# bioinfomaticsCSU/deepsignal

Hardware: AMD Instinct MI355X
Metric: CpG sites/sec (batch=512, k=17, sig=360) (higher is better)
Workload: dtype f32; 1 GPU; configs[1]: 1xMI355X, batch=512, random-init CpG model weights, synthetic (17,360) features, fp32; batch=512, kmer_len=17, signal_len=360

## Files before the change

deepsignal_amd/csrc/ds_engine.cpp:

```cpp
#include "../../include/deepsignal_hip.h"
#include "ds_internal.h"
#include "ds_extract.h"
#include "ds_tsv_device.h"
#include "ds_freq.h"
#include "ds_combine.h"
#include "ds_eval.h"
#include "ds_train.h"
#include "ds_train_signal.h"

#include <algorithm>
#include <cmath>
#include <cstdio>
#include <cstdlib>
#include <cstring>
#include <functional>
#include <map>
#include <string>
#include <vector>

using namespace ds;

namespace {

constexpr int VOCAB = 1024, EMB = 128, HID = 256, NLAYER = 3, NMOD = 11, INC_OUT = 240;
// ... 3 lines not shown

void same_pad(int in, int k, int s, int* out, int* pl)
{
    int o = (in + s - 1) / s;
    int tot = std::max((o - 1) * s + k - in, 0);
    *out = o;
    *pl = tot / 2;
}

struct HostTensor {
    std::vector<int64_t> shape;
    std::vector<float> data;
};

struct PackedGemm {
    float* Bp = nullptr;
    float* bias = nullptr;
    int K = 0, N = 0;
    float* Bps = nullptr;
    float* Bp16 = nullptr;
};

enum OpKind { OP_GEMM, OP_STEM1, OP_MAXPOOL, OP_AVGPOOL, OP_HEAD, OP_FUSED, OP_PACKEV, OP_LSTM, OP_STEM23, OP_HEADF, OP_DENSES, OP_XPROJ };
enum Operands { OPS_FP32, OPS_BF16, OPS_SPLIT };
constexpr KernelClass kFusedKernels[3][3] = {{K_FUSED1, K_FUSED2, K_FUSED3}, {K_FUSEDB1, K_FUSEDB2, K_FUSEDB3}, {K_FUSEDS1, K_FUSEDS2, K_FUSEDS3}};
constexpr KernelClass kStem23Kernels[3] = {K_STEM23, K_STEM23B, K_STEM23S};

struct GemmOp { GemmCfg cfg; int launch_index, total_tiles; };
struct Stem1Op { const float* signals; float* out; };
struct PoolOp { const float* in; float* out; int win, wout, pad, ch; };
struct LstmDiagOp { int launch_index; LstmTile tile; };

struct Op {
    OpKind kind;
    KernelClass kernel;
    Operands operands = OPS_FP32;
    int stream;
    int stage;
    bool after_join = false;
    GemmOp gemm{};
    Stem1Op stem1{};
    PoolOp pool{};
    LstmDiagOp lstm{};
    FusedChain fc{};
    int tm = 0;
    Stem23Args sa{};
    HeadFoldedArgs ha{};
    SplitDense sd{};
    LstmXproj xp{};
    double flops = 0;
    hipEvent_t ev0 = nullptr, ev1 = nullptr;
    bool pending = false;
    int run_launches = 0;
    double run_flops = 0;
};

#define DS_KERNEL_NAME(id, name) name,
const char* const kKernelNames[K_COUNT] = {DS_KERNEL_TABLE(DS_KERNEL_NAME)};
#undef DS_KERNEL_NAME
struct KernelStat {
    int64_t launches = 0;
    double total_ms = 0;
    double flops = 0;
};

struct Stage {
    std::string name;
    int stream = 0;
    int launches = 0;
    double flops_per_site = 0;
    double total_ms = 0;
    int64_t calls = 0;
};

#define DS_SPLIT_DENSE_PARTS 4

struct Plan {
    int n = 0;
    std::vector<GemmLaunch> launches;
    GemmLaunch* d_launches = nullptr;
    std::vector<LstmLaunch> lstm_launches;
    std::vector<Op> ops;
    int fc1_parts = 1;
    hipGraphExec_t graph = nullptr;
    int64_t uses = 0, last_use = 0;
};

enum class Ticket { Idle, Forward, Text, Rows };
using dss::Times;

template <class R>
struct TableRuns {
    R* open = nullptr;
    typename R::Tally ended;
    void close()
    {
        if (!open) return;
        ended.add(open->t);
        delete open;
        open = nullptr;
    }
};
struct Block { char* p = nullptr; size_t cap = 0; };

}

struct Slot {
    hipStream_t s0 = nullptr, s1 = nullptr;
    bool owns_s1 = true;
    hipEvent_t ev_fork = nullptr, ev_join = nullptr;
    float* d_in = nullptr;
    int* d_kmer = nullptr;
    float *d_means = nullptr, *d_stds = nullptr, *d_sanums = nullptr, *d_signals = nullptr;
    float *stem_pool = nullptr, *conv2o = nullptr, *conv3o = nullptr;
    float* modout[NMOD] = {nullptr};
    float *pool2 = nullptr, *pool3 = nullptr;
    float *tmpA = nullptr, *tmpS = nullptr, *tmpB = nullptr;
    float* sigfeat = nullptr;
    float* H[2][NLAYER] = {{nullptr}};
    float* Cst[2][NLAYER] = {{nullptr}};
    float* xproj[2] = {nullptr, nullptr};
    float* hlast[2] = {nullptr, nullptr};
    float *fc1o = nullptr, *logits = nullptr, *act = nullptr;
    int* pred = nullptr;
    float* joint = nullptr;
    char* jsplit = nullptr;

    Ticket ticket = Ticket::Idle;
    int submitted_n = 0;
    char* pin_in = nullptr;
    float* pin_act = nullptr;
    int* pin_pred = nullptr;
    Block pin_reads, d_reads;
    Block d_rows, pin_rows;
    int64_t* pin_rowoff = nullptr;
    char* d_rc = nullptr;
    int* pin_rc = nullptr;
    hipEvent_t rc_ev[2] = {nullptr, nullptr};
    bool rc_selected = false;
    bool rc_timed = false;
    char *pin_text = nullptr, *d_text = nullptr;
    int32_t *d_tres = nullptr, *pin_tres = nullptr;
    hipEvent_t tx_ev[5] = {nullptr, nullptr, nullptr, nullptr, nullptr};
    std::vector<std::pair<const char*, const char*>> text_rows;

    std::map<int, Plan> plans;
    int last_n = 0;
    int last_fc1_parts = 1;
};

#ifndef DS_SPLIT_DENSE_MIN_N
#define DS_SPLIT_DENSE_MIN_N 1
#endif
struct ds_handle {
    ds_config cfg{};
    std::string err;
    int T = 17, S = 360, C = 2;
    int w1 = 0, wa = 0, wb = 0, wc = 0, J = 0, SF = 0;
    int pl_conv1 = 0, pl_pool1 = 0, pl_pool2 = 0, pl_pool3 = 0;
    int B = 512;
    bool is_cnn = true, is_rnn = true, is_base = true;
    bool bf16 = false;
    bool split_dense_narrow = false;
    bool lstm_xproj = false;
    bool lstm_xproj_all = false;
    int split_dense_min_n = DS_SPLIT_DENSE_MIN_N;
    bool split = false;
// ... 942 lines not shown
            if (h->is_rnn) {
                add_seg(G, h->cur->hlast[0], HID, 0, HID);
                add_seg(G, h->cur->hlast[1], HID, 0, HID);
            }
            if (h->is_cnn) add_seg(G, h->cur->sigfeat, h->SF, 0, h->SF);
        }
        add_out(G, h->cur->fc1o, h->J, 0, h->J, 0);
        add_tiles(L, G, fc_cfg);
        P.add_gemm_op(P.tail, st, fc_cfg, L, bf ? (double)h->J / h->JP : 1.0);
    }
    Op op = make_op(OP_HEAD, K_HEAD, 0, stage_id(h, "head", 0));
    op.flops = 2.0 * h->J * h->C * n;
    P.add_op(P.tail, op);
}

int build_plan(ds_handle* h, int n, Plan* plan)
{
    plan->n = n;
    Planner P{h, plan, n, !h->stages_done, h->bf16};
    if (h->is_cnn) plan_signal_model(P);
    plan_event_model(P);
    plan_joint_model(P);

    size_t i = 0, j = 0;
    while (i < P.cnn.size() || j < P.rnn.size()) {
        if (i < P.cnn.size()) plan->ops.push_back(P.cnn[i++]);
        if (j < P.rnn.size()) plan->ops.push_back(P.rnn[j++]);
    }
    for (Op& op : P.tail) { op.after_join = true; plan->ops.push_back(op); }

    void* p = nullptr;
    const auto& LS = plan->launches;
    HIPCHK(h, hipMalloc(&p, LS.size() * sizeof(GemmLaunch)));
    h->allocs.push_back(p);
    plan->d_launches = static_cast<GemmLaunch*>(p);
    HIPCHK(h, hipMemcpy(p, LS.data(), LS.size() * sizeof(GemmLaunch), hipMemcpyHostToDevice));
    return DS_OK;
}

int issue_op(ds_handle* h, Plan& plan, const Op& op, hipStream_t s)
{
    const int n = plan.n;
    const bool bf_rows = op.operands == OPS_BF16;
    switch (op.kind) {
    case OP_GEMM: HIPCHK(h, launch_gemm(op.gemm.cfg, plan.d_launches + op.gemm.launch_index, op.gemm.total_tiles, s)); break;
    case OP_STEM1: HIPCHK(h, launch_stem1(op.stem1.signals, h->stem1_w, h->stem1_b, op.stem1.out, n, h->S, h->w1, h->pl_conv1, h->wa, h->pl_pool1, bf_rows, s)); break;
    case OP_MAXPOOL:
        if (bf_rows) HIPCHK(h, launch_maxpool_s2_bf16(op.pool.in, op.pool.out, n, op.pool.win, op.pool.wout, op.pool.pad, op.pool.ch, s));
        else HIPCHK(h, launch_maxpool_s2(op.pool.in, op.pool.out, n, op.pool.win, op.pool.wout, op.pool.pad, op.pool.ch, s));
        break;
    case OP_AVGPOOL:
        if (bf_rows) HIPCHK(h, launch_avgpool7_bf16(op.pool.in, op.pool.out, n, op.pool.win, op.pool.ch, 256, h->JP, h->is_rnn ? 2 * HID : 0, s));
        else HIPCHK(h, launch_avgpool7(op.pool.in, op.pool.out, n, op.pool.win, op.pool.ch, s));
        break;
    case OP_PACKEV: HIPCHK(h, launch_pack_event_feat_bf16(h->cur->hlast[0], h->cur->hlast[1], h->cur->joint, n, h->JP, 0, s)); break;
    case OP_LSTM:
        if (lstm_tile_is_split(op.lstm.tile)) HIPCHK(h, launch_lstm_cells_split(op.lstm.tile, h->terms, plan.lstm_launches[op.lstm.launch_index], s));
        else HIPCHK(h, launch_lstm_cells(op.lstm.tile, plan.lstm_launches[op.lstm.launch_index], s));
        break;
    case OP_DENSES: HIPCHK(h, launch_dense_split(h->terms, op.sd, s)); break;
    case OP_XPROJ: HIPCHK(h, launch_lstm_xproj(h->terms, op.xp, s)); break;
    case OP_STEM23:
        switch (op.operands) {
        case OPS_FP32: HIPCHK(h, launch_stem23(op.sa, s)); break;
        case OPS_BF16: HIPCHK(h, launch_stem23_bf16(op.sa, s)); break;
        case OPS_SPLIT: HIPCHK(h, launch_stem23_split(h->terms, op.sa, s)); break;
        }
        break;
    case OP_HEADF: HIPCHK(h, launch_head_folded(op.ha, s)); break;
    case OP_FUSED:
        switch (op.operands) {
        case OPS_FP32: HIPCHK(h, launch_inception_fused(op.tm, op.fc, s)); break;
        case OPS_BF16: HIPCHK(h, launch_inception_fused_bf16(op.tm, op.fc, s)); break;
        case OPS_SPLIT: HIPCHK(h, launch_inception_fused_split(h->terms, op.tm, op.fc, s)); break;
        }
        break;
    case OP_HEAD:
        HIPCHK(h, launch_head(h->cur->fc1o, h->fc2, h->cur->logits, h->cur->act, h->cur->pred, n, h->J, h->C, s, plan.fc1_parts, (size_t)h->B * h->J));
        break;
    }
    return DS_OK;
}

int enqueue_forward(ds_handle* h, Plan& plan, int timed)
{
    HIPCHK(h, hipEventRecord(h->cur->ev_fork, h->cur->s0));
    HIPCHK(h, hipStreamWaitEvent(h->cur->s1, h->cur->ev_fork, 0));
    bool joined = false;
    const bool serial = h->serial || timed == 3;
    if (timed == 3) timed = 1;
    Op* head[2] = {nullptr, nullptr};
    auto close_run = [&](int si) -> int {
        if (head[si]) {
            HIPCHK(h, hipEventRecord(head[si]->ev1, si == 0 ? h->cur->s0 : h->cur->s1));
            head[si]->pending = true;
            head[si] = nullptr;
        }
        return DS_OK;
    };
    for (Op& op : plan.ops) {
        const int si = (op.stream == 0 || serial) ? 0 : 1;
        hipStream_t s = si == 0 ? h->cur->s0 : h->cur->s1;
        if (op.after_join && !joined) {
            int rc = close_run(0); if (rc) return rc;
            rc = close_run(1); if (rc) return rc;
            HIPCHK(h, hipEventRecord(h->cur->ev_join, h->cur->s1));
            HIPCHK(h, hipStreamWaitEvent(h->cur->s0, h->cur->ev_join, 0));
            joined = true;
        }
        if (timed && !op.ev0) {
            HIPCHK(h, hipEventCreate(&op.ev0));
            HIPCHK(h, hipEventCreate(&op.ev1));
        }
        if (timed == 2) {
            HIPCHK(h, hipEventRecord(op.ev0, s));
            op.run_launches = 1; op.run_flops = op.flops;
        } else if (timed == 1) {
            if (head[si] && head[si]->kernel != op.kernel) { int rc = close_run(si); if (rc) return rc; }
            if (!head[si]) {
                head[si] = &op;
                op.run_launches = 0; op.run_flops = 0;
                HIPCHK(h, hipEventRecord(op.ev0, s));
            }
            head[si]->run_launches += 1;
            head[si]->run_flops += op.flops;
        }
        int rc = issue_op(h, plan, op, s);
        if (rc) return rc;
        if (timed == 2) {
            HIPCHK(h, hipEventRecord(op.ev1, s));
            op.pending = true;
        }
    }
    { int rc = close_run(0); if (rc) return rc; rc = close_run(1); if (rc) return rc; }
    if (!joined) {
        HIPCHK(h, hipEventRecord(h->cur->ev_join, h->cur->s1));
        HIPCHK(h, hipStreamWaitEvent(h->cur->s0, h->cur->ev_join, 0));
    }
    return DS_OK;
}

int collect_stage_times(ds_handle* h)
{
    for (Slot& sl : h->slots)
      for (auto& kv : sl.plans)
        for (Op& op : kv.second.ops) {
            if (!op.pending) continue;
            HIPCHK(h, hipEventSynchronize(op.ev1));
            float ms = 0;
            HIPCHK(h, hipEventElapsedTime(&ms, op.ev0, op.ev1));
            h->stages[op.stage].total_ms += ms;
            KernelStat& K = h->kstat[op.kernel];
            K.launches += op.run_launches; K.total_ms += ms; K.flops += op.run_flops;
            op.pending = false;
        }
    return DS_OK;
}

void destroy_plan(ds_handle* h, Plan& p)
{
    if (p.graph) hipGraphExecDestroy(p.graph);
    for (Op& op : p.ops) { if (op.ev0) hipEventDestroy(op.ev0); if (op.ev1) hipEventDestroy(op.ev1); }
    if (p.d_launches) {
        hipFree(p.d_launches);
        auto it = std::find(h->allocs.begin(), h->allocs.end(), (void*)p.d_launches);
        if (it != h->allocs.end()) h->allocs.erase(it);
    }
    p.graph = nullptr; p.d_launches = nullptr; p.ops.clear();
}

constexpr size_t MAX_PLANS_PER_SLOT = 24;

int get_plan(ds_handle* h, int n, Plan** out)
{
    auto& plans = h->cur->plans;
    auto it = plans.find(n);
    if (it == plans.end()) {
        if (plans.size() >= MAX_PLANS_PER_SLOT && !h->profiling) {
            auto victim = plans.end();
            for (auto jt = plans.begin(); jt != plans.end(); ++jt)
                if (jt->first != h->B && (victim == plans.end() || jt->second.last_use < victim->second.last_use)) victim = jt;
            if (victim != plans.end()) {
                HIPCHK(h, hipStreamSynchronize(h->cur->s0));
                HIPCHK(h, hipStreamSynchronize(h->cur->s1));
                destroy_plan(h, victim->second);
                plans.erase(victim);
            }
        }
        Plan p;
        int rc = build_plan(h, n, &p);
        if (rc) return rc;
        it = plans.emplace(n, std::move(p)).first;
        h->stages_done = true;
    }
    it->second.uses += 1;
    it->second.last_use = ++h->plan_tick;
    *out = &it->second;
    return DS_OK;
}

int ensure_graph(ds_handle* h, Plan& plan)
{
    if (plan.graph) return DS_OK;
    hipGraph_t g = nullptr;
    HIPCHK(h, hipStreamBeginCapture(h->cur->s0, hipStreamCaptureModeThreadLocal));
    int rc = enqueue_forward(h, plan, 0);
    hipError_t e = hipStreamEndCapture(h->cur->s0, &g);
    if (rc) { if (g) hipGraphDestroy(g); return rc; }
    if (e != hipSuccess) return fail(h, DS_ERR_HIP, std::string("hipStreamEndCapture: ") + hipGetErrorString(e));
    e = hipGraphInstantiate(&plan.graph, g, nullptr, nullptr, 0);
    hipGraphDestroy(g);
    if (e != hipSuccess) return fail(h, DS_ERR_HIP, std::string("hipGraphInstantiate: ") + hipGetErrorString(e));
    return DS_OK;
}

int run_resident(ds_handle* h, int n)
{
    Plan* plan = nullptr;
    int rc = get_plan(h, n, &plan);
    if (rc) return rc;
    h->cur->last_n = n;
    h->cur->last_fc1_parts = plan->fc1_parts;
    if (h->profiling) {
        rc = collect_stage_times(h);
        if (rc) return rc;
        rc = enqueue_forward(h, *plan, h->profiling);
        if (rc) return rc;
        for (Stage& S : h->stages) S.calls += 1;
        return DS_OK;
    }
    if (h->use_graph && (plan->graph || n == h->B || plan->uses >= 2)) {
        rc = ensure_graph(h, *plan);
        if (rc) return rc;
        HIPCHK(h, hipGraphLaunch(plan->graph, h->cur->s0));
        return DS_OK;
    }
    return enqueue_forward(h, *plan, 0);
}

void prepare_slots(ds_handle* h)
{
    if (!h->use_graph || h->debug || h->serial) return;
    Slot* keep = h->cur;
    const std::string err_before = h->err;
    for (Slot& sl : h->slots) {
        h->cur = &sl;
        Plan* plan = nullptr;
        int rc = get_plan(h, h->B, &plan);
        if (!rc) { plan->uses = 0; rc = ensure_graph(h, *plan); }
        if (rc) {
            fprintf(stderr, "deepsignal_amd: preparing a slot's full-batch plan failed (%s); plans will be built at the first forward\n",
                    h->err.c_str());
            h->err = err_before;
            break;
        }
    }
    h->cur = keep;
}

}

namespace {
template <class F>
auto guarded(ds_handle* h, F&& body) -> decltype(body())
{
    try {
        return body();
    } catch (const std::bad_alloc&) {
        return fail(h, DS_ERR_NOMEM, "out of host memory");
    } catch (const std::exception& e) {
        return fail(h, DS_ERR_INVALID, std::string("internal error: ") + e.what());
    } catch (...) {
        return fail(h, DS_ERR_INVALID, "internal error");
    }
}

template <class R, class Begin>
int open_run(ds_handle* h, TableRuns<R> ds_handle::*runs, const char* call, Begin begin)
{
    if (!h) return DS_ERR_INVALID;
    TableRuns<R>& r = h->*runs;
    if (r.open) return fail(h, DS_ERR_INVALID, std::string(R::ROUTE) + "_" + call + ": a run is open on this handle (" + R::ROUTE + "_end first)");
    r.open = new R();
    std::string err;
    const int rc = begin(*r.open, &err);
    if (rc == DS_OK) return DS_OK;
    delete r.open;
    r.open = nullptr;
    return fail(h, rc, err);
}

template <class R, class Call>
auto in_run(ds_handle* h, TableRuns<R> ds_handle::*runs, const char* call, Call body, const char* opener = "begin")
    -> decltype(body(std::declval<R&>(), (std::string*)nullptr))
{
    if (!h) return DS_ERR_INVALID;
    R* r = (h->*runs).open;
    if (!r) return fail(h, DS_ERR_INVALID, std::string(R::ROUTE) + "_" + call + ": no run is open (" + R::ROUTE + "_" + opener + " first)");
    std::string err;
    const auto rc = body(*r, &err);
    return rc < 0 ? fail(h, (int)rc, err) : rc;
}

template <class R>
int end_run(ds_handle* h, TableRuns<R> ds_handle::*runs)
{
    if (!h) return DS_ERR_INVALID;
    (h->*runs).close();
    return DS_OK;
}
}

extern "C" {

const char* ds_version(void)
{
    return "deepsignal_amd 0.5 (gfx950; fp32 MFMA, bf16 conv + FC and bf16_all operand modes; bf16x3 = fp32 operands as three bf16 "
           "terms, six products per MAC, in: conv_layer2 / 3, the eleven inception modules, the BiLSTM cells' recurrent and lower-layer products, dense(J, J) of the three-step "
           "joint model; fp16x2 = the same scope on two fp16 terms, three products per MAC, operands within +-65504)";
}

const char* ds_last_error(const ds_handle* h) { return h ? h->err.c_str() : g_create_error.c_str(); }

static int ds_create_impl(const ds_config* cfg, ds_handle** out)
{
    if (!cfg || !out) return fail(nullptr, DS_ERR_INVALID, "ds_create: null argument");
    *out = nullptr;
    if (!(cfg->is_cnn || cfg->is_rnn))
        return fail(nullptr, DS_ERR_INVALID, "at least one of is_cnn/is_rnn should be True");
    if (cfg->precision != DS_PRECISION_FP32 && cfg->precision != DS_PRECISION_BF16 && cfg->precision != DS_PRECISION_BF16_ALL &&
        cfg->precision != DS_PRECISION_BF16X3 && cfg->precision != DS_PRECISION_FP16X2)
        return fail(nullptr, DS_ERR_UNSUPPORTED, "precision must be DS_PRECISION_FP32, DS_PRECISION_BF16, DS_PRECISION_BF16_ALL, DS_PRECISION_BF16X3 or DS_PRECISION_FP16X2");
    if (cfg->precision == DS_PRECISION_BF16X3 && (cfg->reserved[2] & DS_TUNE_NO_FUSED))
        return fail(nullptr, DS_ERR_UNSUPPORTED, "DS_PRECISION_BF16X3 runs the fused inception kernels only (DS_TUNE_NO_FUSED asks for the layer-granular fp32 path)");
    if (cfg->precision == DS_PRECISION_FP16X2 && (cfg->reserved[2] & DS_TUNE_NO_FUSED))
        return fail(nullptr, DS_ERR_UNSUPPORTED, "DS_PRECISION_FP16X2 runs the fused inception kernels only (DS_TUNE_NO_FUSED asks for the layer-granular fp32 path)");
    if (cfg->kmer_len < 1 || cfg->kmer_len > 255 || (cfg->kmer_len & 1) == 0)
        return fail(nullptr, DS_ERR_INVALID, "kmer_len must be odd and in [1,255]");
    if (cfg->signal_len < 16 || cfg->class_num < 1 || cfg->class_num > 16)
        return fail(nullptr, DS_ERR_INVALID, "bad signal_len/class_num");
    if (cfg->signal_len > DS_MAX_SIGNAL_LEN)
        return fail(nullptr, DS_ERR_UNSUPPORTED, "signal_len " + std::to_string(cfg->signal_len) + " > DS_MAX_SIGNAL_LEN (" +
                    std::to_string(DS_MAX_SIGNAL_LEN) + "): the stem's window does not fit the 64 KB of dynamic LDS it may use");
    int ndev = 0;
    hipError_t e = hipGetDeviceCount(&ndev);
    if (e != hipSuccess || ndev <= 0)
        return fail(nullptr, DS_ERR_HIP, std::string("no HIP device available: ") + hipGetErrorString(e));
    if (cfg->device < 0 || cfg->device >= ndev) return fail(nullptr, DS_ERR_INVALID, "device ordinal out of range");
    ds_handle* h = new ds_handle();
    h->cfg = *cfg;
    h->slots.resize(1);
    h->cur = &h->slots[0];
    h->T = cfg->kmer_len; h->S = cfg->signal_len; h->C = cfg->class_num;
    h->B = cfg->max_batch > 0 ? cfg->max_batch : 512;
    same_pad(h->S, 7, 2, &h->w1, &h->pl_conv1);
    same_pad(h->w1, 3, 2, &h->wa, &h->pl_pool1);
    same_pad(h->wa, 3, 2, &h->wb, &h->pl_pool2);
    same_pad(h->wb, 3, 2, &h->wc, &h->pl_pool3);
    h->is_cnn = cfg->is_cnn != 0; h->is_rnn = cfg->is_rnn != 0; h->is_base = cfg->is_base != 0;
    h->SF = h->wc * INC_OUT;
    h->J = (h->is_rnn ? 2 * HID : 0) + (h->is_cnn ? h->SF : 0);
    h->bf16 = cfg->precision == DS_PRECISION_BF16 || cfg->precision == DS_PRECISION_BF16_ALL;
    h->lstm_bf16 = cfg->precision == DS_PRECISION_BF16_ALL && h->is_rnn;
    h->split = cfg->precision == DS_PRECISION_BF16X3 || cfg->precision == DS_PRECISION_FP16X2;
    h->terms = cfg->precision == DS_PRECISION_FP16X2 ? TERMS_FP16X2 : TERMS_BF16X3;
    const int32_t flags = cfg->reserved[2];
    h->no_fused = (flags & DS_TUNE_NO_FUSED) != 0;
    h->serial = (flags & DS_TUNE_SERIAL) != 0;
    h->serial_modules = (flags & DS_TUNE_NO_CHAIN) != 0;
    h->shared_s1 = (flags & DS_TUNE_SHARED_EVENT_STREAM) != 0 && !h->serial;
    if (h->shared_s1) h->use_graph = false;
    h->fold_fc = !(flags & DS_TUNE_NO_FOLD_FC) && cfg->reserved[0] == 0 && cfg->class_num <= 16;
    h->lstm_variant = cfg->reserved[3];
    if (cfg->reserved[4] > 0) h->fuse_max_spt = cfg->reserved[4];
    if (cfg->reserved[5] > 0) h->fuse_min_tiles = cfg->reserved[5];
    if (cfg->reserved[6] > 0) h->split_dense_min_n = cfg->reserved[6];
    h->split_dense_narrow = (flags & DS_TUNE_SPLIT_DENSE_NARROW) != 0;
    h->lstm_xproj = h->split && h->is_rnn && !(flags & DS_TUNE_NO_LSTM_XPROJ);
    h->lstm_xproj_all = h->lstm_xproj && (flags & DS_TUNE_LSTM_XPROJ_ALL);
    h->Bp32 = (h->B + 31) / 32 * 32;
    h->JP = (h->J + 31) / 32 * 32;
    h->debug = cfg->reserved[0] != 0;
#define CK(expr) do { hipError_t e_ = (expr); if (e_ != hipSuccess) { fail(nullptr, DS_ERR_HIP, std::string(#expr) + ": " + hipGetErrorString(e_)); ds_destroy(h); return DS_ERR_HIP; } } while (0)
    CK(hipSetDevice(cfg->device));
    CK(configure_fused_kernels());
    CK(configure_split_kernels());
    int nslots = cfg->reserved[1] > 0 ? cfg->reserved[1] : (h->B <= 1024 && !h->bf16 ? 8 : 4);
    nslots = std::max(1, std::min(nslots, 16));
    h->slots.resize(nslots);
    int rc = DS_OK;
    for (Slot& sl : h->slots) {
        h->cur = &sl;
        CK(hipStreamCreateWithFlags(&sl.s0, hipStreamNonBlocking));
        if (h->shared_s1 && &sl != &h->slots[0]) { sl.s1 = h->slots[0].s1; sl.owns_s1 = false; }
        else CK(hipStreamCreateWithFlags(&sl.s1, hipStreamNonBlocking));
        CK(hipEventCreateWithFlags(&sl.ev_fork, hipEventDisableTiming));
        CK(hipEventCreateWithFlags(&sl.ev_join, hipEventDisableTiming));
        if (!rc) rc = alloc_workspace(h);
    }
    h->cur = &h->slots[0];
#undef CK
    if (!rc) {
        if (!rc && (flags & DS_TUNE_DEBUG_STAMPS)) {
            rc = dalloc(h, &h->dbg_stamps, (size_t)NMOD * 1024 * 16);
            if (!rc) hipMemset(h->dbg_stamps, 0, (size_t)NMOD * 1024 * 16 * 8);
            if (!rc) rc = dalloc(h, &h->dbg_lstm, (size_t)32 * 1024 * 8);
            if (!rc) hipMemset(h->dbg_lstm, 0, (size_t)32 * 1024 * 8 * 8);
        }
    }
    if (rc) { g_create_error = h->err; ds_destroy(h); return rc; }
    *out = h;
    return DS_OK;
}

void ds_destroy(ds_handle* h)
{
    if (!h) return;
    hipSetDevice(h->cfg.device);
    for (Slot& sl : h->slots) {
        if (sl.s0) hipStreamSynchronize(sl.s0);
        if (sl.s1) hipStreamSynchronize(sl.s1);
    }
    for (Slot& sl : h->slots) {
        for (auto& kv : sl.plans) {
            if (kv.second.graph) hipGraphExecDestroy(kv.second.graph);
            for (Op& op : kv.second.ops) { if (op.ev0) hipEventDestroy(op.ev0); if (op.ev1) hipEventDestroy(op.ev1); }
        }
        for (void* p : {(void*)sl.pin_in, (void*)sl.pin_act , (void*)sl.pin_rowoff, (void*)sl.pin_rc,
                        (void*)sl.pin_text, (void*)sl.pin_tres, (void*)sl.pin_reads.p, (void*)sl.pin_rows.p})
            if (p) hipHostFree(p);
        for (void* p : {(void*)sl.d_rc, (void*)sl.d_text, (void*)sl.d_tres, (void*)sl.d_reads.p, (void*)sl.d_rows.p})
            if (p) hipFree(p);
        for (hipEvent_t e : sl.tx_ev) if (e) hipEventDestroy(e);
        for (hipEvent_t e : sl.rc_ev) if (e) hipEventDestroy(e);
        if (sl.ev_fork) hipEventDestroy(sl.ev_fork);
        if (sl.ev_join) hipEventDestroy(sl.ev_join);
        if (sl.s0) hipStreamDestroy(sl.s0);
        if (sl.s1 && sl.owns_s1) hipStreamDestroy(sl.s1);
    }
    h->freq.close();
    h->combine.close();
    h->eval.close();
    delete h->train;
    for (void* p : h->allocs) hipFree(p);
    (void)hipGetLastError();
    delete h;
}

static int ds_set_tensor_impl(ds_handle* h, const char* name, const float* data, const int64_t* shape, int32_t ndim)
{
    if (!h || !name || !data || !shape || ndim < 1 || ndim > 8) return fail(h, DS_ERR_INVALID, "ds_set_tensor: bad argument");
    if (h->finalized) return fail(h, DS_ERR_INVALID, "weights already finalized");
    HostTensor t;
    int64_t cnt = 1;
    for (int i = 0; i < ndim; ++i) { t.shape.push_back(shape[i]); cnt *= shape[i]; }
    if (cnt <= 0) return fail(h, DS_ERR_INVALID, "ds_set_tensor: empty tensor");
    t.data.assign(data, data + cnt);
    h->host[name] = std::move(t);
    return DS_OK;
}

static int ds_finalize_weights_impl(ds_handle* h)
{
    if (!h) return DS_ERR_INVALID;
    if (h->finalized) return fail(h, DS_ERR_INVALID, "weights already finalized");
    hipSetDevice(h->cfg.device);
    const size_t allocs_before = h->allocs.size();
    int rc = finalize_weights(h);
    h->weight_allocs.assign(h->allocs.begin() + allocs_before, h->allocs.end());
    if (!rc) prepare_slots(h);
    return rc;
}

static int ds_load_weights_impl(ds_handle* h, const char* path)
{
    if (!h || !path) return fail(h, DS_ERR_INVALID, "ds_load_weights: bad argument");
    FILE* f = fopen(path, "rb");
    if (!f) return fail(h, DS_ERR_IO, std::string("cannot open ") + path);
    auto bad = [&](const char* why) { fclose(f); return fail(h, DS_ERR_IO, std::string(path) + ": " + why); };
    char magic[8];
    uint32_t nt = 0;
    if (fread(magic, 1, 8, f) != 8 || memcmp(magic, "DSAMDW01", 8) != 0) return bad("not a DSAMDW01 file");
    if (fread(&nt, 4, 1, f) != 1 || nt > 100000) return bad("bad tensor count");
    struct Meta { std::string name; std::vector<int64_t> shape; uint64_t off, nbytes; };
    std::vector<Meta> metas(nt);
    if (fseek(f, 0, SEEK_END) != 0) return bad("cannot seek");
    const long fsize_l = ftell(f);
    if (fsize_l < 12 || fseek(f, 12, SEEK_SET) != 0) return bad("cannot seek");
    const uint64_t fsize = (uint64_t)fsize_l;
    for (auto& m : metas) {
        uint16_t ln = 0; uint8_t nd = 0;
        if (fread(&ln, 2, 1, f) != 1) return bad("truncated header");
        m.name.resize(ln);
        if (ln && fread(&m.name[0], 1, ln, f) != ln) return bad("truncated header");
        if (fread(&nd, 1, 1, f) != 1 || nd > 8) return bad("truncated header");
        for (int i = 0; i < nd; ++i) { uint32_t d = 0; if (fread(&d, 4, 1, f) != 1) return bad("truncated header"); m.shape.push_back(d); }
        if (fread(&m.off, 8, 1, f) != 1 || fread(&m.nbytes, 8, 1, f) != 1) return bad("truncated header");
        const uint64_t max_elems = (uint64_t)1 << 32;
        uint64_t cnt = 1;
        for (int64_t d : m.shape) {
            if (d <= 0 || (uint64_t)d > max_elems / cnt) return bad("bad tensor shape");
            cnt *= (uint64_t)d;
        }
        if (m.nbytes != cnt * 4) return bad("tensor byte count does not match its shape");
        if (m.off > fsize || m.nbytes > fsize - m.off) return bad("tensor payload lies outside the file");
    }
    for (auto& m : metas) {
        HostTensor t;
        t.shape = m.shape;
        t.data.resize(m.nbytes / 4);
        if (fseek(f, (long)m.off, SEEK_SET) != 0 || fread(t.data.data(), 1, m.nbytes, f) != m.nbytes) return bad("truncated payload");
        h->host[m.name] = std::move(t);
    }
    fclose(f);
    return ds_finalize_weights(h);
}

static int ds_forward_device_impl(ds_handle* h, int32_t n, const int32_t* d_kmer, const float* d_means, const float* d_stds,
                      const float* d_sanums, const float* d_signals, float* d_act, int32_t* d_pred)
{
    if (!h) return DS_ERR_INVALID;
    if (!h->finalized) return fail(h, DS_ERR_INVALID, "weights not loaded");
    if (n < 0 || n > h->B) return fail(h, DS_ERR_INVALID, "n exceeds max_batch");
    if (h->rc_fine)
        return fail(h, DS_ERR_UNSUPPORTED, "ds_forward_device is not available on a handle with a recheck attached (ds_set_recheck)");
    if (n == 0) return DS_OK;
    if (!d_kmer || !d_means || !d_stds || !d_sanums || !d_signals || !d_act || !d_pred)
        return fail(h, DS_ERR_INVALID, "null buffer");
    HIPCHK(h, hipSetDevice(h->cfg.device));
    h->cur = &h->slots[h->profiling ? 0 : (h->next_slot++ % h->slots.size())];
    HIPCHK(h, launch_gather_inputs(d_kmer, d_means, d_stds, d_sanums, d_signals, h->cur->d_in, n, h->T, h->S, h->B, h->cur->s0));
    int rc = run_resident(h, n);
    if (rc) return rc;
    HIPCHK(h, launch_scatter_outputs(h->cur->act, h->cur->pred, d_act, d_pred, n, h->C, h->cur->s0));
    return DS_OK;
}

int ds_sync(ds_handle* h)
{
    if (!h) return DS_ERR_INVALID;
    for (Slot& sl : h->slots) {
        HIPCHK(h, hipStreamSynchronize(sl.s0));
        HIPCHK(h, hipStreamSynchronize(sl.s1));
    }
    if (h->profiling) return collect_stage_times(h);
    return DS_OK;
}

static int enqueue_recheck(ds_handle* h, Slot& sl, int n);
static int finish_recheck(ds_handle* h, Slot& sl, int n, float* act, int32_t* pred);


static int idle_slot(ds_handle* h, const char* who, Slot** sl)
{
    HIPCHK(h, hipSetDevice(h->cfg.device));
    const int si = (int)(h->next_slot % h->slots.size());
    if (h->slots[si].ticket != Ticket::Idle)
        return fail(h, DS_ERR_INVALID, std::string(who) + ": every slot is in flight; wait the oldest ticket first");
    *sl = &h->slots[si];
    return DS_OK;
}

static void hold(ds_handle* h, Slot& sl, Ticket kind, int n, int32_t* ticket)
{
    sl.ticket = kind;
    sl.submitted_n = n;
    *ticket = (int32_t)(&sl - h->slots.data());
}

static void release(Slot& sl) { sl.ticket = Ticket::Idle; sl.submitted_n = 0; }

static bool tickets_in_flight(const ds_handle* h)
{
    return std::any_of(h->slots.begin(), h->slots.end(), [](const Slot& sl) { return sl.ticket != Ticket::Idle; });
}

static int ticket_slot(ds_handle* h, const char* who, int32_t ticket, Ticket kind, Slot** sl, int* n)
{
    static const char* const carries[] = {"nothing", "forward", "text rows", "rows"};
    if (ticket < 0 || ticket >= (int)h->slots.size() || h->slots[ticket].ticket != kind)
        return fail(h, DS_ERR_INVALID, std::string(who) + ": no " + carries[(int)kind] + " in flight for this ticket");
    HIPCHK(h, hipSetDevice(h->cfg.device));
    *sl = &h->slots[ticket];
    *n = (*sl)->submitted_n;
    return DS_OK;
}

static int stage_host_inputs(ds_handle* h, Slot& sl, int nparts, const int32_t* counts, const int32_t* const* kmer, const float* const* means,
                             const float* const* stds, const float* const* sanums, const float* const* signals)
{
    const InLayout L = in_layout(h);
    if (!sl.pin_in) HIPCHK(h, hipHostMalloc((void**)&sl.pin_in, L.total, hipHostMallocDefault));
    char* dev = reinterpret_cast<char*>(sl.d_in);
    size_t n = 0;
    for (int i = 0; i < nparts; ++i) {
        const size_t c = (size_t)counts[i];
        if (!c) continue;
        const void* src[5] = {kmer[i], means[i], stds[i], sanums[i], signals[i]};
        for (int k = 0; k < 5; ++k) memcpy(sl.pin_in + L.at[k] + n * L.row[k], src[k], c * L.row[k]);
        n += c;
    }
    if (n == (size_t)h->B) {
        HIPCHK(h, hipMemcpyAsync(dev, sl.pin_in, L.total, hipMemcpyHostToDevice, sl.s0));
        return DS_OK;
    }
    for (int k = 0; k < 5; ++k)
        HIPCHK(h, hipMemcpyAsync(dev + L.at[k], sl.pin_in + L.at[k], n * L.row[k], hipMemcpyHostToDevice, sl.s0));
    return DS_OK;
}

static int enqueue_forward_on(ds_handle* h, Slot& sl, int n)
{
    if (!sl.pin_act) {
        HIPCHK(h, hipHostMalloc((void**)&sl.pin_act, ((size_t)h->B * h->C + h->B) * 4, hipHostMallocDefault));
        sl.pin_pred = reinterpret_cast<int*>(sl.pin_act + (size_t)h->B * h->C);
// ... 1480 lines not shown
```

deepsignal_amd/csrc/ds_internal.h:

```cpp
#pragma once
#include <hip/hip_runtime.h>
#include <stdint.h>

namespace ds {

constexpr int KC = 16;
constexpr int MAX_SEG = 6;
constexpr int MAX_OUT = 6;
constexpr int MAX_PROB = 8;

struct ASeg {
    const float* base;
    int ld;
    int row_shift;
    int klen;
    int pad_;
};

struct OSeg {
    float* base;
    const float* add;
    int ld;
    int add_ld;
    int col0;
// ... 133 lines not shown

hipError_t launch_gemm(GemmCfg cfg, const GemmLaunch* d_launch, int total_tiles, hipStream_t s);

struct FusedArgs {
    const float* X;
    float* Y;
    int n_sites, W, cin, spt;
    int pool_win, pool_pad;
    const float* Bp1;
    const float* bias1;
    const float *Bp3b, *bias3b, *Bp4b, *bias4b, *Bp5b, *bias5b, *Bp5c, *bias5c;
    const float *Bp3r, *Bp4r;
    const float* Bp1r;
    unsigned long long* dbg;
    int write_rows;
};

size_t inception_fused_lds_bytes(int tm, int W, int spt);
hipError_t configure_fused_kernels();
constexpr int FUSED_CHAIN_MAX = 5;
struct FusedChain {
    FusedArgs m[FUSED_CHAIN_MAX];
    int nmod;
};
hipError_t launch_inception_fused_bf16(int tm, const FusedChain& c, hipStream_t s);
hipError_t launch_inception_fused(int tm, const FusedChain& c, hipStream_t s);
size_t inception_fused_bf16_lds_bytes(int tm, int W, int spt);
hipError_t launch_inception_fused_split(TermFormat fmt, int tm, const FusedChain& c, hipStream_t s);
size_t inception_fused_split_lds_bytes(int tm, int W, int spt);
hipError_t configure_split_kernels();
hipError_t launch_lstm_cells_split(LstmTile tile, TermFormat fmt, const LstmLaunch& L, hipStream_t s);
struct SplitDense {
    const float* seg[3];
    int len[3];
    char* A;
    const char* Bp;
    float* C;
    int n, N, mtiles, ntiles, ntiles_alloc, ksteps, kg_stride;
    int splits;
    size_t part_stride;
    bool wide;
};
hipError_t launch_dense_split(TermFormat fmt, const SplitDense& d, hipStream_t s);

struct Stem23Args {
    const float* X;
    float* Y;
    float* C2;
    const float *Bp2, *bias2;
    const float *Bp3, *bias3;
    int n_sites, W, spt;
};
hipError_t launch_stem23(const Stem23Args& a, hipStream_t s);
hipError_t launch_stem23_split(TermFormat fmt, const Stem23Args& a, hipStream_t s);
size_t stem23_split_lds_bytes(int W, int spt);
size_t stem23_lds_bytes(int W, int spt);
hipError_t launch_stem23_bf16(const Stem23Args& a, hipStream_t s);
size_t stem23_bf16_lds_bytes(int W, int spt);
constexpr size_t STEM23_MAX_LDS = 80 * 1024;
hipError_t launch_stem1(const float* signals, const float* w7x64, const float* bias64, float* out,
                        int n, int signal_len, int w1, int pad_l_conv, int wa, int pad_l_pool, int out_bf16, hipStream_t s);
hipError_t launch_maxpool_s2_bf16(const float* in, float* out, int n, int win, int wout, int pad_l, int ch_ld, hipStream_t s);
hipError_t launch_avgpool7_bf16(const float* in, float* joint, int n, int w, int ch, int ld_in, int joint_ld, int joint_off,
                                hipStream_t s);
hipError_t launch_pack_event_feat_bf16(const float* hfw, const float* hbw, float* joint, int n, int joint_ld, int src_bf16,
                                       hipStream_t s);
hipError_t launch_maxpool_s2(const float* in, float* out, int n, int win, int wout, int pad_l, int ch, hipStream_t s);
hipError_t launch_avgpool7(const float* in, float* out, int n, int w, int ch, hipStream_t s);
hipError_t launch_head(const float* fc1, const float* w2, float* logits, float* act, int* pred,
                       int n, int J, int class_num, hipStream_t s, int nparts = 1, size_t part_stride = 0);
struct HeadFoldedArgs {
    const float* seg[3];
    int len[3];
    int nseg;
    const float* w;
    int bf16;
    int pitch[3];
    float *logits, *act;
    int* pred;
    int n, C;
};
hipError_t launch_head_folded(const HeadFoldedArgs& a, hipStream_t s);
hipError_t launch_gather_inputs(const int* kmer, const float* means, const float* stds, const float* lens, const float* signals,
                                float* block, int n, int T, int S, int B, hipStream_t s);
hipError_t launch_scatter_outputs(const float* act, const int* pred, float* act_out, int* pred_out, int n, int C, hipStream_t s);
struct RecheckArgs {
    const float* act;
    const float* in;
    float* out;
    int* count;
    int* index;
    float margin;
    int n, C, T, S, B;
};
hipError_t launch_recheck_select(const RecheckArgs& a, hipStream_t s);
hipError_t launch_embed_table(const float* emb, const float* kernel, float* table, int vocab, int esize, int ncol, hipStream_t s);

}
```

deepsignal_amd/csrc/ds_kernels.hip:

```cpp
#include "ds_device.h"

namespace ds {


constexpr int DR_SLOTS = 4;
constexpr int DR_DIST = 3;
constexpr int DR_STAGE = 6 * 256;
constexpr int DR_A_FLOATS = 2 * 128 * (KC + 4);
constexpr int DR_LDS_FLOATS = DR_A_FLOATS + DR_SLOTS * DR_STAGE + 2 * 256;
constexpr int DR_SOLO_PAD_BYTES = 56 * 1024;

__device__ __forceinline__ void dr_gload4(v4f& dst, unsigned voff, const void* sbase)
{
    asm volatile("global_load_dwordx4 %0, %1, %2" : "=&v"(dst) : "v"(voff), "s"(sbase) : "memory");
}
template <int E> __device__ __forceinline__ float dr_elem(const v4f& v) { return E == 0 ? v.x : E == 1 ? v.y : E == 2 ? v.z : v.w; }

__device__ __forceinline__ void dense_ring_loop(const GemmProblem& P, float* smem, int m0, int tid, int lane, int wave,
                                                int t0, int t1, int t2, floatx16 (&acc)[1][3])
{
    constexpr int LDA = KC + 4;
    const int nchunks = P.K / KC;
    if (nchunks <= 0) return;
    float* const ring = smem + DR_A_FLOATS;
// ... 2276 lines not shown
#pragma unroll
    for (int c = 0; c < 16; ++c) accv[c] = 0.0f;
    int koff = 0;
    if (a.bf16) {
        for (int sg = 0; sg < a.nseg; ++sg) {
        const float4* x8 = reinterpret_cast<const float4*>(reinterpret_cast<const unsigned short*>(a.seg[sg]) + (size_t)site * a.pitch[sg]);
        for (int k8 = tid; k8 < (a.len[sg] >> 3); k8 += 256) {
            const float4 raw = x8[k8];
            const unsigned u[4] = {__float_as_uint(raw.x), __float_as_uint(raw.y), __float_as_uint(raw.z), __float_as_uint(raw.w)};
            const float* w = a.w + (size_t)(koff + k8 * 8) * C;
            if (C == 2) {
#pragma unroll
                for (int e = 0; e < 4; ++e) {
                    const float x0 = __uint_as_float(u[e] << 16), x1 = __uint_as_float(u[e] & 0xffff0000u);
                    const float4 wv = *reinterpret_cast<const float4*>(w + 4 * e);
                    accv[0] = fmaf(x0, wv.x, fmaf(x1, wv.z, accv[0]));
                    accv[1] = fmaf(x0, wv.y, fmaf(x1, wv.w, accv[1]));
                }
            } else {
#pragma unroll
                for (int e = 0; e < 4; ++e) {
                    const float x0 = __uint_as_float(u[e] << 16), x1 = __uint_as_float(u[e] & 0xffff0000u);
#pragma unroll
                    for (int c = 0; c < 16; ++c)
                        if (c < C) accv[c] += x0 * w[(2 * e) * C + c] + x1 * w[(2 * e + 1) * C + c];
                }
            }
        }
        koff += a.len[sg];
        }
    } else
    for (int sg = 0; sg < a.nseg; ++sg) {
        const int len = a.len[sg];
        const float4* x4 = reinterpret_cast<const float4*>(a.seg[sg] + (size_t)site * len);
        for (int k4 = tid; k4 < (len >> 2); k4 += 256) {
            const float4 x = x4[k4];
            const float* w = a.w + (size_t)(koff + k4 * 4) * C;
            if (C == 2) {
                const float4 wa = *reinterpret_cast<const float4*>(w);
                const float4 wb = *reinterpret_cast<const float4*>(w + 4);
                accv[0] = fmaf(x.x, wa.x, fmaf(x.y, wa.z, fmaf(x.z, wb.x, fmaf(x.w, wb.z, accv[0]))));
                accv[1] = fmaf(x.x, wa.y, fmaf(x.y, wa.w, fmaf(x.z, wb.y, fmaf(x.w, wb.w, accv[1]))));
            } else {
#pragma unroll
                for (int c = 0; c < 16; ++c)
                    if (c < C) accv[c] += x.x * w[c] + x.y * w[C + c] + x.z * w[2 * C + c] + x.w * w[3 * C + c];
            }
        }
        koff += len;
    }
#pragma unroll
    for (int c = 0; c < 16; ++c) {
        if (c >= C) break;
        float v = accv[c];
#pragma unroll
        for (int off = 32; off > 0; off >>= 1) v += __shfl_xor(v, off);
        if (lane == 0) part[wave][c] = v;
    }
    __syncthreads();
    if (tid == 0) {
        float best = 0.0f;
        int bi = 0;
        for (int c = 0; c < C; ++c) {
            const float v = (part[0][c] + part[1][c]) + (part[2][c] + part[3][c]);
            const float sgm = sigmoidf_(v);
            a.logits[(size_t)site * C + c] = v;
            a.act[(size_t)site * C + c] = sgm;
            if (c == 0 || sgm > best) { best = sgm; bi = c; }
        }
        a.pred[site] = bi;
    }
}

hipError_t launch_head_folded(const HeadFoldedArgs& a, hipStream_t s)
{
    if (a.n <= 0) return hipSuccess;
    hipLaunchKernelGGL(head_folded_kernel, dim3(a.n), dim3(256), 0, s, a);
    return hipGetLastError();
}

__global__ __launch_bounds__(256) void gather_inputs_kernel(const int* __restrict__ kmer, const float* __restrict__ means,
                                                            const float* __restrict__ stds, const float* __restrict__ lens,
                                                            const float* __restrict__ signals, float* __restrict__ block,
                                                            int n, int T, int S, int B)
{
    const long nt = (long)n * T, ns = (long)n * S, total = 4 * nt + ns;
    const long bt = (long)B * T;
    for (long i = (long)blockIdx.x * 256 + threadIdx.x; i < total; i += (long)gridDim.x * 256) {
        if (i < nt) reinterpret_cast<int*>(block)[i] = kmer[i];
        else if (i < 2 * nt) block[bt + (i - nt)] = means[i - nt];
        else if (i < 3 * nt) block[2 * bt + (i - 2 * nt)] = stds[i - 2 * nt];
        else if (i < 4 * nt) block[3 * bt + (i - 3 * nt)] = lens[i - 3 * nt];
        else block[4 * bt + (i - 4 * nt)] = signals[i - 4 * nt];
    }
}

__global__ __launch_bounds__(256) void scatter_outputs_kernel(const float* __restrict__ act, const int* __restrict__ pred,
                                                              float* __restrict__ act_out, int* __restrict__ pred_out, int n, int C)
{
    const int total = n * C + n;
    for (int i = blockIdx.x * 256 + threadIdx.x; i < total; i += gridDim.x * 256) {
        if (i < n * C) act_out[i] = act[i];
        else pred_out[i - n * C] = pred[i - n * C];
    }
}

hipError_t launch_gather_inputs(const int* kmer, const float* means, const float* stds, const float* lens, const float* signals,
                                float* block, int n, int T, int S, int B, hipStream_t s)
{
    if (n <= 0) return hipSuccess;
    const long total = (long)n * (4 * T + S);
    const int grid = (int)std::min<long>((total + 1023) / 1024, 1024);
    hipLaunchKernelGGL(gather_inputs_kernel, dim3(grid), dim3(256), 0, s, kmer, means, stds, lens, signals, block, n, T, S, B);
    return hipGetLastError();
}

hipError_t launch_scatter_outputs(const float* act, const int* pred, float* act_out, int* pred_out, int n, int C, hipStream_t s)
{
    if (n <= 0) return hipSuccess;
    hipLaunchKernelGGL(scatter_outputs_kernel, dim3((n * (C + 1) + 255) / 256), dim3(256), 0, s, act, pred, act_out, pred_out, n, C);
    return hipGetLastError();
}

__global__ __launch_bounds__(256) void maxpool_s2_bf16_kernel(const float4* __restrict__ in, float4* __restrict__ out,
                                                               long total, int win, int wout, int pad_l, int ch8)
{
    for (long i = blockIdx.x * (long)blockDim.x + threadIdx.x; i < total; i += (long)gridDim.x * blockDim.x) {
        const int c = (int)(i % ch8);
        const long r = i / ch8;
        const int wo = (int)(r % wout);
        const long site = r / wout;
        float4 m = make_float4(0.0f, 0.0f, 0.0f, 0.0f);
#pragma unroll
        for (int t = 0; t < 3; ++t) {
            const int wi = 2 * wo + t - pad_l;
            if (wi >= 0 && wi < win) m = bf8max_relu(m, in[(site * win + wi) * ch8 + c]);
        }
        out[i] = m;
    }
}

hipError_t launch_maxpool_s2_bf16(const float* in, float* out, int n, int win, int wout, int pad_l, int ch_ld, hipStream_t s)
{
    const long total = (long)n * wout * (ch_ld / 8);
    if (total <= 0) return hipSuccess;
    const int blocks = (int)((total + 255) / 256 < 8192 ? (total + 255) / 256 : 8192);
    hipLaunchKernelGGL(maxpool_s2_bf16_kernel, dim3(blocks), dim3(256), 0, s, (const float4*)in, (float4*)out, total, win,
                       wout, pad_l, ch_ld / 8);
    return hipGetLastError();
}

__global__ __launch_bounds__(256) void avgpool7_bf16_kernel(const float4* __restrict__ in, unsigned short* __restrict__ out,
                                                             long total, int w, int ch8, int ld_in8, long out_ld, int out_off)
{
    for (long i = blockIdx.x * (long)blockDim.x + threadIdx.x; i < total; i += (long)gridDim.x * blockDim.x) {
        const int c = (int)(i % ch8);
        const long r = i / ch8;
        const int wo = (int)(r % w);
        const long site = r / w;
        float a[8] = {0, 0, 0, 0, 0, 0, 0, 0};
        int cnt = 0;
        for (int t = -3; t <= 3; ++t) {
            const int wi = wo + t;
            if (wi < 0 || wi >= w) continue;
            const float4 v = in[(site * w + wi) * ld_in8 + c];
            const unsigned u[4] = {__float_as_uint(v.x), __float_as_uint(v.y), __float_as_uint(v.z), __float_as_uint(v.w)};
#pragma unroll
            for (int q = 0; q < 4; ++q) {
                a[2 * q] += __uint_as_float(u[q] << 16);
                a[2 * q + 1] += __uint_as_float(u[q] & 0xffff0000u);
            }
            ++cnt;
        }
        const float d = (float)cnt;
        unsigned o[4];
#pragma unroll
        for (int q = 0; q < 4; ++q) o[q] = pack_bf2(a[2 * q] / d, a[2 * q + 1] / d);
        *reinterpret_cast<uint4*>(out + site * out_ld + out_off + ((long)wo * ch8 + c) * 8) = make_uint4(o[0], o[1], o[2], o[3]);
    }
}

hipError_t launch_avgpool7_bf16(const float* in, float* joint, int n, int w, int ch, int ld_in, int joint_ld, int joint_off,
                                hipStream_t s)
{
    const long total = (long)n * w * (ch / 8);
    if (total <= 0) return hipSuccess;
    const int blocks = (int)((total + 255) / 256 < 8192 ? (total + 255) / 256 : 8192);
    hipLaunchKernelGGL(avgpool7_bf16_kernel, dim3(blocks), dim3(256), 0, s, (const float4*)in, (unsigned short*)joint, total, w,
                       ch / 8, ld_in / 8, (long)joint_ld, joint_off);
    return hipGetLastError();
}

template <bool SRC_BF>
__global__ __launch_bounds__(256) void pack_event_feat_bf16_kernel(const float* __restrict__ hfw, const float* __restrict__ hbw,
                                                                    unsigned short* __restrict__ joint, int n, long joint_ld)
{
// ... 50 lines not shown
```

Baseline: 454,000 sites/s.

## Split forward graph per stream and gather only the inputs each branch needs

The single captured forward graph becomes two per-stream graphs: an event/RNN branch on s1 and a signal branch on s0, with post-join ops issued eagerly. Input gathering is split by column range so the RNN features are copied on s1 right after the fork, and signal columns are skipped when the model is not CNN. The default slot count also drops to 4 unless split or folded FC is enabled. The aim is to let the two branches start independently and cut unneeded copies, at the cost of more host launches (two graph launches plus eager tail ops) and more event sync per call.

```diff
diff --git a/deepsignal_amd/csrc/ds_engine.cpp b/deepsignal_amd/csrc/ds_engine.cpp
--- a/deepsignal_amd/csrc/ds_engine.cpp
+++ b/deepsignal_amd/csrc/ds_engine.cpp
@@ -109,7 +109,9 @@
     std::vector<LstmLaunch> lstm_launches;
     std::vector<Op> ops;
     int fc1_parts = 1;
-    hipGraphExec_t graph = nullptr;
+    hipGraphExec_t graph_ev = nullptr, graph_sig = nullptr;
+    bool captured = false;
+    bool ev_on_s1 = false;
     int64_t uses = 0, last_use = 0;
 };
 
@@ -1218,10 +1220,23 @@
     return DS_OK;
 }
 
-int enqueue_forward(ds_handle* h, Plan& plan, int timed)
+int fork_event_stream(ds_handle* h)
 {
     HIPCHK(h, hipEventRecord(h->cur->ev_fork, h->cur->s0));
     HIPCHK(h, hipStreamWaitEvent(h->cur->s1, h->cur->ev_fork, 0));
+    return DS_OK;
+}
+
+int join_event_stream(ds_handle* h)
+{
+    HIPCHK(h, hipEventRecord(h->cur->ev_join, h->cur->s1));
+    HIPCHK(h, hipStreamWaitEvent(h->cur->s0, h->cur->ev_join, 0));
+    return DS_OK;
+}
+
+int enqueue_forward(ds_handle* h, Plan& plan, int timed, bool forked)
+{
+    if (!forked) { int rc = fork_event_stream(h); if (rc) return rc; }
     bool joined = false;
     const bool serial = h->serial || timed == 3;
     if (timed == 3) timed = 1;
@@ -1240,8 +1255,7 @@
         if (op.after_join && !joined) {
             int rc = close_run(0); if (rc) return rc;
             rc = close_run(1); if (rc) return rc;
-            HIPCHK(h, hipEventRecord(h->cur->ev_join, h->cur->s1));
-            HIPCHK(h, hipStreamWaitEvent(h->cur->s0, h->cur->ev_join, 0));
+            rc = join_event_stream(h); if (rc) return rc;
             joined = true;
         }
         if (timed && !op.ev0) {
@@ -1269,10 +1283,7 @@
         }
     }
     { int rc = close_run(0); if (rc) return rc; rc = close_run(1); if (rc) return rc; }
-    if (!joined) {
-        HIPCHK(h, hipEventRecord(h->cur->ev_join, h->cur->s1));
-        HIPCHK(h, hipStreamWaitEvent(h->cur->s0, h->cur->ev_join, 0));
-    }
+    if (!joined) return join_event_stream(h);
     return DS_OK;
 }
 
@@ -1293,16 +1304,24 @@
     return DS_OK;
 }
 
+void destroy_graphs(Plan& p)
+{
+    if (p.graph_ev) hipGraphExecDestroy(p.graph_ev);
+    if (p.graph_sig) hipGraphExecDestroy(p.graph_sig);
+    p.graph_ev = p.graph_sig = nullptr;
+    p.captured = false;
+}
+
 void destroy_plan(ds_handle* h, Plan& p)
 {
-    if (p.graph) hipGraphExecDestroy(p.graph);
+    destroy_graphs(p);
     for (Op& op : p.ops) { if (op.ev0) hipEventDestroy(op.ev0); if (op.ev1) hipEventDestroy(op.ev1); }
     if (p.d_launches) {
         hipFree(p.d_launches);
         auto it = std::find(h->allocs.begin(), h->allocs.end(), (void*)p.d_launches);
         if (it != h->allocs.end()) h->allocs.erase(it);
     }
-    p.graph = nullptr; p.d_launches = nullptr; p.ops.clear();
+    p.d_launches = nullptr; p.ops.clear();
 }
 
 constexpr size_t MAX_PLANS_PER_SLOT = 24;
@@ -1335,22 +1354,56 @@
     return DS_OK;
 }
 
-int ensure_graph(ds_handle* h, Plan& plan)
-{
-    if (plan.graph) return DS_OK;
+bool graphs_split(const ds_handle* h) { return h->is_rnn && !h->serial; }
+bool event_ops_on_s1(const ds_handle* h) { return graphs_split(h) && h->profiling != 3; }
+
+int capture_branch(ds_handle* h, Plan& plan, int si, hipGraphExec_t* out)
+{
+    const bool split = plan.ev_on_s1;
+    auto mine = [&](const Op& op) { return !op.after_join && ((op.stream == 1 && split) ? 1 : 0) == si; };
+    if (std::none_of(plan.ops.begin(), plan.ops.end(), mine)) return DS_OK;
+    hipStream_t s = si == 0 ? h->cur->s0 : h->cur->s1;
     hipGraph_t g = nullptr;
-    HIPCHK(h, hipStreamBeginCapture(h->cur->s0, hipStreamCaptureModeThreadLocal));
-    int rc = enqueue_forward(h, plan, 0);
-    hipError_t e = hipStreamEndCapture(h->cur->s0, &g);
+    HIPCHK(h, hipStreamBeginCapture(s, hipStreamCaptureModeThreadLocal));
+    int rc = DS_OK;
+    for (const Op& op : plan.ops)
+        if (mine(op) && (rc = issue_op(h, plan, op, s))) break;
+    hipError_t e = hipStreamEndCapture(s, &g);
     if (rc) { if (g) hipGraphDestroy(g); return rc; }
     if (e != hipSuccess) return fail(h, DS_ERR_HIP, std::string("hipStreamEndCapture: ") + hipGetErrorString(e));
-    e = hipGraphInstantiate(&plan.graph, g, nullptr, nullptr, 0);
+    e = hipGraphInstantiate(out, g, nullptr, nullptr, 0);
     hipGraphDestroy(g);
     if (e != hipSuccess) return fail(h, DS_ERR_HIP, std::string("hipGraphInstantiate: ") + hipGetErrorString(e));
     return DS_OK;
 }
 
-int run_resident(ds_handle* h, int n)
+int ensure_graphs(ds_handle* h, Plan& plan)
+{
+    if (plan.captured) return DS_OK;
+    plan.ev_on_s1 = graphs_split(h);
+    int rc = capture_branch(h, plan, 1, &plan.graph_ev);
+    if (!rc) rc = capture_branch(h, plan, 0, &plan.graph_sig);
+    if (rc) { destroy_graphs(plan); return rc; }
+    plan.captured = true;
+    return DS_OK;
+}
+
+int replay_forward(ds_handle* h, Plan& plan, bool forked)
+{
+    if (forked && !(plan.ev_on_s1 && plan.graph_ev))
+        return fail(h, DS_ERR_INVALID, "internal error: the forward was forked to the event stream, its captured graphs were not");
+    if (plan.graph_ev) {
+        if (!forked) { int rc = fork_event_stream(h); if (rc) return rc; }
+        HIPCHK(h, hipGraphLaunch(plan.graph_ev, h->cur->s1));
+    }
+    if (plan.graph_sig) HIPCHK(h, hipGraphLaunch(plan.graph_sig, h->cur->s0));
+    if (plan.graph_ev || forked) { int rc = join_event_stream(h); if (rc) return rc; }
+    for (const Op& op : plan.ops)
+        if (op.after_join) { int rc = issue_op(h, plan, op, h->cur->s0); if (rc) return rc; }
+    return DS_OK;
+}
+
+int run_resident(ds_handle* h, int n, bool forked = false)
 {
     Plan* plan = nullptr;
     int rc = get_plan(h, n, &plan);
@@ -1360,18 +1413,17 @@
     if (h->profiling) {
         rc = collect_stage_times(h);
         if (rc) return rc;
-        rc = enqueue_forward(h, *plan, h->profiling);
+        rc = enqueue_forward(h, *plan, h->profiling, forked);
         if (rc) return rc;
         for (Stage& S : h->stages) S.calls += 1;
         return DS_OK;
     }
-    if (h->use_graph && (plan->graph || n == h->B || plan->uses >= 2)) {
-        rc = ensure_graph(h, *plan);
+    if (h->use_graph && (plan->captured || n == h->B || plan->uses >= 2)) {
+        rc = ensure_graphs(h, *plan);
         if (rc) return rc;
-        HIPCHK(h, hipGraphLaunch(plan->graph, h->cur->s0));
-        return DS_OK;
-    }
-    return enqueue_forward(h, *plan, 0);
+        return replay_forward(h, *plan, forked);
+    }
+    return enqueue_forward(h, *plan, 0, forked);
 }
 
 void prepare_slots(ds_handle* h)
@@ -1383,7 +1435,7 @@
         h->cur = &sl;
         Plan* plan = nullptr;
         int rc = get_plan(h, h->B, &plan);
-        if (!rc) { plan->uses = 0; rc = ensure_graph(h, *plan); }
+        if (!rc) { plan->uses = 0; rc = ensure_graphs(h, *plan); }
         if (rc) {
             fprintf(stderr, "deepsignal_amd: preparing a slot's full-batch plan failed (%s); plans will be built at the first forward\n",
                     h->err.c_str());
@@ -1521,7 +1573,8 @@
     CK(hipSetDevice(cfg->device));
     CK(configure_fused_kernels());
     CK(configure_split_kernels());
-    int nslots = cfg->reserved[1] > 0 ? cfg->reserved[1] : (h->B <= 1024 && !h->bf16 ? 8 : 4);
+    const bool eight = h->B <= 1024 && !h->bf16 && (h->split || h->fold_fc);
+    int nslots = cfg->reserved[1] > 0 ? cfg->reserved[1] : (eight ? 8 : 4);
     nslots = std::max(1, std::min(nslots, 16));
     h->slots.resize(nslots);
     int rc = DS_OK;
@@ -1559,7 +1612,7 @@
     }
     for (Slot& sl : h->slots) {
         for (auto& kv : sl.plans) {
-            if (kv.second.graph) hipGraphExecDestroy(kv.second.graph);
+            destroy_graphs(kv.second);
             for (Op& op : kv.second.ops) { if (op.ev0) hipEventDestroy(op.ev0); if (op.ev1) hipEventDestroy(op.ev1); }
         }
         for (void* p : {(void*)sl.pin_in, (void*)sl.pin_act , (void*)sl.pin_rowoff, (void*)sl.pin_rc,
@@ -1665,8 +1718,17 @@
         return fail(h, DS_ERR_INVALID, "null buffer");
     HIPCHK(h, hipSetDevice(h->cfg.device));
     h->cur = &h->slots[h->profiling ? 0 : (h->next_slot++ % h->slots.size())];
-    HIPCHK(h, launch_gather_inputs(d_kmer, d_means, d_stds, d_sanums, d_signals, h->cur->d_in, n, h->T, h->S, h->B, h->cur->s0));
-    int rc = run_resident(h, n);
+    const bool forked = event_ops_on_s1(h);
+    const int ev_end = 4 * h->T, row_end = 4 * h->T + h->S;
+    int rc = DS_OK;
+    if (forked) {
+        if ((rc = fork_event_stream(h))) return rc;
+        HIPCHK(h, launch_gather_inputs(d_kmer, d_means, d_stds, d_sanums, d_signals, h->cur->d_in, n, h->T, h->S, h->B, 0, ev_end, h->cur->s1));
+    }
+    const int s0_from = (forked || !h->is_rnn) ? ev_end : 0, s0_to = h->is_cnn ? row_end : ev_end;
+    if (s0_from < s0_to)
+        HIPCHK(h, launch_gather_inputs(d_kmer, d_means, d_stds, d_sanums, d_signals, h->cur->d_in, n, h->T, h->S, h->B, s0_from, s0_to, h->cur->s0));
+    rc = run_resident(h, n, forked);
     if (rc) return rc;
     HIPCHK(h, launch_scatter_outputs(h->cur->act, h->cur->pred, d_act, d_pred, n, h->C, h->cur->s0));
     return DS_OK;
diff --git a/deepsignal_amd/csrc/ds_internal.h b/deepsignal_amd/csrc/ds_internal.h
--- a/deepsignal_amd/csrc/ds_internal.h
+++ b/deepsignal_amd/csrc/ds_internal.h
@@ -239,7 +239,7 @@
 };
 hipError_t launch_head_folded(const HeadFoldedArgs& a, hipStream_t s);
 hipError_t launch_gather_inputs(const int* kmer, const float* means, const float* stds, const float* lens, const float* signals,
-                                float* block, int n, int T, int S, int B, hipStream_t s);
+                                float* block, int n, int T, int S, int B, int col_lo, int col_hi, hipStream_t s);
 hipError_t launch_scatter_outputs(const float* act, const int* pred, float* act_out, int* pred_out, int n, int C, hipStream_t s);
 struct RecheckArgs {
     const float* act;
diff --git a/deepsignal_amd/csrc/ds_kernels.hip b/deepsignal_amd/csrc/ds_kernels.hip
--- a/deepsignal_amd/csrc/ds_kernels.hip
+++ b/deepsignal_amd/csrc/ds_kernels.hip
@@ -2382,11 +2382,11 @@
 __global__ __launch_bounds__(256) void gather_inputs_kernel(const int* __restrict__ kmer, const float* __restrict__ means,
                                                             const float* __restrict__ stds, const float* __restrict__ lens,
                                                             const float* __restrict__ signals, float* __restrict__ block,
-                                                            int n, int T, int S, int B)
-{
-    const long nt = (long)n * T, ns = (long)n * S, total = 4 * nt + ns;
+                                                            int n, int T, int S, int B, long lo, long hi)
+{
+    const long nt = (long)n * T;
     const long bt = (long)B * T;
-    for (long i = (long)blockIdx.x * 256 + threadIdx.x; i < total; i += (long)gridDim.x * 256) {
+    for (long i = lo + (long)blockIdx.x * 256 + threadIdx.x; i < hi; i += (long)gridDim.x * 256) {
         if (i < nt) reinterpret_cast<int*>(block)[i] = kmer[i];
         else if (i < 2 * nt) block[bt + (i - nt)] = means[i - nt];
         else if (i < 3 * nt) block[2 * bt + (i - 2 * nt)] = stds[i - 2 * nt];
@@ -2406,12 +2406,12 @@
 }
 
 hipError_t launch_gather_inputs(const int* kmer, const float* means, const float* stds, const float* lens, const float* signals,
-                                float* block, int n, int T, int S, int B, hipStream_t s)
-{
-    if (n <= 0) return hipSuccess;
-    const long total = (long)n * (4 * T + S);
-    const int grid = (int)std::min<long>((total + 1023) / 1024, 1024);
-    hipLaunchKernelGGL(gather_inputs_kernel, dim3(grid), dim3(256), 0, s, kmer, means, stds, lens, signals, block, n, T, S, B);
+                                float* block, int n, int T, int S, int B, int col_lo, int col_hi, hipStream_t s)
+{
+    if (n <= 0 || col_lo < 0 || col_hi > 4 * T + S || col_lo >= col_hi) return hipSuccess;
+    const long lo = (long)n * col_lo, hi = (long)n * col_hi;
+    const int grid = (int)std::min<long>((hi - lo + 1023) / 1024, 1024);
+    hipLaunchKernelGGL(gather_inputs_kernel, dim3(grid), dim3(256), 0, s, kmer, means, stds, lens, signals, block, n, T, S, B, lo, hi);
     return hipGetLastError();
 }
 
```

After: 461,500 sites/s, median of 6. 1.02x the previous value.
